# nilsfriess/MultigridMC

Measured on AMD Instinct MI355X. Metric: MGMC V-cycle samples/sec + fine-smoother HBM GB/s, 512³ lattice, 1/2/4/8 GPUs, higher is better.
Workload: dtype f64

## Files before the change

multigridmc_amd/csrc/mgmc_capi.hip:

```cpp
#include "mgmc_internal.hpp"

namespace mgmc_host {
std::mutex g_err_mutex;
std::string g_last_error;
std::atomic<int> g_live_handles{0};
void set_global_error(const std::string& s) {
    std::lock_guard<std::mutex> lock(g_err_mutex);
    g_last_error = s;
}
}

namespace {
constexpr int LDS_POISON_DOUBLES = 80 * 1024 / 8;
__global__ void __launch_bounds__(1024) k_lds_poison() {
    extern __shared__ double lds[];
    const double nan = __builtin_nan("");
    for (int q = threadIdx.x; q < LDS_POISON_DOUBLES; q += blockDim.x) lds[q] = nan;
    __syncthreads();
    if (lds[(threadIdx.x * 7) % LDS_POISON_DOUBLES] == 0.0) asm volatile("" ::: "memory");
}
__global__ void __launch_bounds__(256) k_poison_interior(Layout L, double* __restrict__ x) {
    const int i = blockIdx.x * blockDim.x + threadIdx.x + 1;
    const int j = blockIdx.y + 1;
    const int k = L.dim == 3 ? (int)blockIdx.z + 1 : 0;
// ... 22 lines not shown
    g.seed_hi = (uint32_t)(h->seed >> 32);
    return g;
}

RngKey chain_key_host(const GibbsArg& g, int c) {
    RngKey k = g.key;
    if (c) k.k1 = (g.chain0 + (uint32_t)c) ^ g.seed_hi;
    return k;
}
template <class T>
T* chain_ptr(T* v, const Level& lv, int c) {
    return v ? v + (long long)c * lv.L.nstore : v;
}

template <int DIM, int NPTS, bool NOISE>
void launch_sweep_t(const Level& lv, double* x, const double* f, const GibbsArg& g0, int direction,
                    hipStream_t s) {
    const Layout& L = lv.L;
    const int nc = lv.spec.ncolours;
    dim3 block(64, 4, 1);
    for (int cc = 0; cc < nc; ++cc) {
        GibbsArg g = g0;
        g.colour = (direction == MGMC_FORWARD) ? cc : nc - 1 - cc;
        if (NPTS == 5 || NPTS == 7) {
            dim3 grid = grid3(L.nx / 2, L.ny - 1, DIM == 3 ? L.nz - 1 : 1, block);
            hipLaunchKernelGGL((k_sweep_rb<DIM, NPTS, NOISE>), grid, block, 0, s, L, x, f, lv.S, g);
        } else {
            dim3 grid = grid3(L.nx / 2, L.ny / 2, DIM == 3 ? L.nz / 2 : 1, block);
            hipLaunchKernelGGL((k_sweep_mc<DIM, NPTS, NOISE>), grid, block, 0, s, L, x, f, lv.S, g);
        }
    }
}

void launch_fsweep(const Level& lv, double* x, const double* f, const GibbsArg& g0, int direction, bool noise,
                   hipStream_t s) {
    const Layout& L = lv.L;
    const int nc = lv.F.scheme, dim = lv.spec.dim;
    const int st = nc == 9 || nc == 27 ? 3 : 2;
    dim3 block(64, 4, 1);
    dim3 grid = nc == 2 ? grid3(L.nx / 2, L.ny - 1, dim == 3 ? L.nz - 1 : 1, block)
                        : grid3((L.nx - 1 + st - 1) / st, (L.ny - 1 + st - 1) / st,
                                dim == 3 ? (L.nz - 1 + st - 1) / st : 1, block);
    for (int cc = 0; cc < nc; ++cc) {
        GibbsArg g = g0;
        g.colour = (direction == MGMC_FORWARD) ? cc : nc - 1 - cc;
        if (dim == 3) {
            if (noise) hipLaunchKernelGGL((k_fsweep<3, true>), grid, block, 0, s, L, x, f, lv.F, g);
            else hipLaunchKernelGGL((k_fsweep<3, false>), grid, block, 0, s, L, x, f, lv.F, g);
        } else {
            if (noise) hipLaunchKernelGGL((k_fsweep<2, true>), grid, block, 0, s, L, x, f, lv.F, g);
            else hipLaunchKernelGGL((k_fsweep<2, false>), grid, block, 0, s, L, x, f, lv.F, g);
        }
    }
}

void launch_sweep(const Level& lv, double* x, const double* f, const GibbsArg& g0, int direction, bool noise,
                  hipStream_t s, int nch) {
    if (nch > 1) {
        for (int c = 0; c < nch; ++c) {
            GibbsArg g = g0;
            g.key = chain_key_host(g0, c);
            launch_sweep(lv, chain_ptr(x, lv, c), chain_ptr(f, lv, c), g, direction, noise, s, 1);
        }
        return;
    }
    const GibbsArg& g = g0;
    if (lv.field) {
        launch_fsweep(lv, x, f, g, direction, noise, s);
        return;
    }
    const int dim = lv.spec.dim, np = lv.spec.npoints;
#define DISPATCH(D, P)                                                       \
    if (dim == D && np == P) {                                               \
        if (noise)                                                           \
            launch_sweep_t<D, P, true>(lv, x, f, g, direction, s);           \
        else                                                                 \
            launch_sweep_t<D, P, false>(lv, x, f, g, direction, s);          \
        return;                                                              \
    }
    DISPATCH(3, 7) DISPATCH(3, 27) DISPATCH(2, 5) DISPATCH(2, 9)
#undef DISPATCH
}

template <int XP, int TY, int NT, int MINW = 1>
void launch_zsweep_t(const Level& lv, ZSweepArgs a, bool prolong, hipStream_t s, int nch, bool fz) {
    a.ntx = (lv.L.nx / 2) / XP;
    a.nty = (lv.L.ny - 1 + TY - 1) / TY;
    a.ntz = (lv.L.nz - 1 + a.tz - 1) / a.tz;
    const int ntiles = a.ntx * a.nty * (a.zpairs ? (a.ntz + 1) / 2 * 2 : a.ntz);
    const int nb = (ntiles + 7) / 8 * 8;
    const size_t lds = zsweep_lds_bytes(XP, TY, prolong);
    int ex;
    const bool pow2 = std::isnormal(a.alpha) && std::frexp(std::fabs(a.alpha), &ex) == 0.5 && ex > -900 && ex < 900;
    const dim3 grid(nb, 1, nch);
    const bool lrf = a.lr.e != nullptr;
    if (fz && !lrf) {
        if (prolong && pow2)
            hipLaunchKernelGGL((k_zsweep_rb7<XP, TY, NT, 2, MINW, false, true>), grid, dim3(NT), lds, s, a);
        else if (prolong)
            hipLaunchKernelGGL((k_zsweep_rb7<XP, TY, NT, 1, MINW, false, true>), grid, dim3(NT), lds, s, a);
        else
            hipLaunchKernelGGL((k_zsweep_rb7<XP, TY, NT, 0, MINW, false, true>), grid, dim3(NT), lds, s, a);
        return;
    }
    if (prolong && pow2 && lrf)
        hipLaunchKernelGGL((k_zsweep_rb7<XP, TY, NT, 2, MINW, true>), grid, dim3(NT), lds, s, a);
    else if (prolong && pow2)
        hipLaunchKernelGGL((k_zsweep_rb7<XP, TY, NT, 2, MINW>), grid, dim3(NT), lds, s, a);
    else if (prolong && lrf)
        hipLaunchKernelGGL((k_zsweep_rb7<XP, TY, NT, 1, MINW, true>), grid, dim3(NT), lds, s, a);
    else if (prolong)
        hipLaunchKernelGGL((k_zsweep_rb7<XP, TY, NT, 1, MINW>), grid, dim3(NT), lds, s, a);
    else if (lrf)
        hipLaunchKernelGGL((k_zsweep_rb7<XP, TY, NT, 0, MINW, true>), grid, dim3(NT), lds, s, a);
    else
        hipLaunchKernelGGL((k_zsweep_rb7<XP, TY, NT, 0, MINW>), grid, dim3(NT), lds, s, a);
}

static int zsweep_depth(const Level& lv, int ty, int tzmax) {
    const long long tiles_xy = (long long)((lv.L.nx / 2) / ZS_XP) * ((lv.L.ny - 1 + ty - 1) / ty);
    int tz = tzmax;
    while (tz > 8 && 4 * tiles_xy * ((lv.L.nz - 1 + tz - 1) / tz) < 3LL * 2 * lv.num_cu) tz /= 2;
    return tz;
}

static int zsweep_plain_rows(const Level& lv, int nch) {
    const int tz = zsweep_depth(lv, ZS_TY, ZS_TZ);
    auto ntiles = [&](int ty) {
        const long long nz = (lv.L.nz - 1 + tz - 1) / tz;
        return (long long)((lv.L.nx / 2) / ZS_XP) * ((lv.L.ny - 1 + ty - 1) / ty) * ((nz + 1) / 2 * 2) * nch;
    };
    const long long slots = 2LL * lv.num_cu;
    return (ZS_TYP != ZS_TY && ZS_NTP == ZS_NT && ntiles(ZS_TY) < slots && ntiles(ZS_TYP) <= slots) ? ZS_TYP : ZS_TY;
}

void launch_zsweep(const Level& lv, const double* xin, double* xout, const double* f, const GibbsArg& g0,
                   int direction, const Level* coarse, const double* xc, double alpha, hipStream_t s, int nch = 1,
                   const LRRhsArg* lr = nullptr, bool fzero = false) {
    ZSweepArgs a;
    a.lr = lr ? *lr : LRRhsArg{nullptr};
    a.cs = lv.L.nstore;
    a.csc = coarse ? coarse->L.nstore : 0;
    a.L = lv.L;
    a.xin = xin;
    a.xout = xout;
    a.f = f;
    a.xc = xc;
    a.Lc = coarse ? coarse->L : lv.L;
    a.alpha = alpha;
    a.S = lv.S;
    a.G = g0;
    a.G.colour = (direction == MGMC_FORWARD) ? 0 : 1;
    a.zpairs = 0;
    if (coarse) {
        a.tz = zsweep_depth(lv, ZS_TYP, ZS_TZP);
        launch_zsweep_t<ZS_XP, ZS_TYP, ZS_NTP, ZS_MINWP>(lv, a, true, s, nch, fzero);
        return;
    }
    a.tz = zsweep_depth(lv, ZS_TY, ZS_TZ);
    a.zpairs = 1;
    if (zsweep_plain_rows(lv, nch) != ZS_TY) {
        launch_zsweep_t<ZS_XP, ZS_TYP, ZS_NTP, ZS_MINWP>(lv, a, false, s, nch, fzero);
        return;
    }
    launch_zsweep_t<ZS_XP, ZS_TY, ZS_NT, ZS_MINW>(lv, a, false, s, nch, fzero);
}

bool pairs_eligible(const LevelSpec& sp, const Layout& L) {
    return (sp.npoints == 27 || sp.npoints == 9) && L.nx / 2 >= 1 && L.nx / 2 <= 256 && L.nx % 2 == 0;
}

bool quads_eligible(const LevelSpec& sp, const Layout& L, uint32_t paths) {
    if (!pairs_eligible(sp, L) || (paths & PATH_NO_QUADS)) return false;
    return sp.dim == 2 || L.nx / 2 <= tune::QUADS_MAXPAIR;
}

void launch_rb2d(const Level& lv, const double* xin, double* xout, const double* f, const GibbsArg& g, int direction,
                 bool noise, hipStream_t s, int nch = 1) {
    const int ntx = (lv.L.nx - 1 + RB2_TW - 1) / RB2_TW, nty = (lv.L.ny - 1 + RB2_TH - 1) / RB2_TH;
    const int c1 = direction == MGMC_FORWARD ? 0 : 1;
    const dim3 grid(ntx * nty, 1, nch), block(RB2_NT);
    const long long cs = lv.L.nstore;
    if (noise)
        hipLaunchKernelGGL((k_rb2d<true>), grid, block, 0, s, lv.L, xin, xout, f, lv.S, g, c1, ntx, cs);
    else
        hipLaunchKernelGGL((k_rb2d<false>), grid, block, 0, s, lv.L, xin, xout, f, lv.S, g, c1, ntx, cs);
}

bool jsweep_eligible(const LevelSpec& sp, const Layout& L, uint32_t paths) {
    return sp.dim == 3 && sp.npoints == 27 && (L.nx == 256 || L.nx == 512) &&
           L.ny >= 2 && L.nz >= 2 &&
           !(paths & PATH_NO_JSWEEP);
}


void launch_jsweep(const Level& lv, const double* xin, double* xout, const double* f, const GibbsArg& g, int direction,
                   hipStream_t s, int nch, bool xzero = false) {
    JSweepArgs a;
    a.cs = lv.L.nstore;
    a.L = lv.L;
    a.xo = xin;
    a.xout = xout;
    a.f = f;
    a.S = lv.S;
    a.G = g;
    const int np = lv.L.nx / 2;
    const size_t lds = jsweep_lds_bytes(np);
    const bool fwd = direction == MGMC_FORWARD;
    for (int h = 0; h < 2; ++h) {
        const JSweepPlan p = jsweep_plan(lv.L, fwd, h, lv.num_cu, lds, tune::JS_ROUNDS);
        if (p.nk == 0) continue;
        a.kp = p.kp;
        a.jA = p.jA;
        a.nsteps = p.nsteps;
        a.nk = p.nk;
        a.spc = p.spc;
        a.nchunk = p.nchunk;
        a.xz = h == 0 ? xin : xout;
        const dim3 grid(p.nb, 1, nch), block(2 * np);
#define MGMC_JS_LAUNCH_XZ(NPV, SYMV, XZ)                                                            \
    do {                                                                                            \
        if (fwd) hipLaunchKernelGGL((k_jsweep_half<NPV, false, SYMV, XZ>), grid, block, lds, s, a); \
        else hipLaunchKernelGGL((k_jsweep_half<NPV, true, SYMV, XZ>), grid, block, lds, s, a);      \
    } while (0)
#define MGMC_JS_LAUNCH(NPV, SYMV)                                 \
    do {                                                          \
        if (!xzero) MGMC_JS_LAUNCH_XZ(NPV, SYMV, 0);              \
        else if (h == 0) MGMC_JS_LAUNCH_XZ(NPV, SYMV, 1);         \
        else MGMC_JS_LAUNCH_XZ(NPV, SYMV, 2);                     \
    } while (0)
        if (np == 256) {
            MGMC_JS_LAUNCH(256, false);
        } else if (lv.sym) {
            MGMC_JS_LAUNCH(128, true);
        } else {
            MGMC_JS_LAUNCH(128, false);
        }
#undef MGMC_JS_LAUNCH
#undef MGMC_JS_LAUNCH_XZ
    }
}

void launch_quads(const Level& lv, const double* xin, double* xout, const double* f, const GibbsArg& g, int direction,
                  hipStream_t s, int nch = 1, bool xzero = false, const double2* zb = nullptr) {
    if (lv.jsweep) {
        launch_jsweep(lv, xin, xout, f, g, direction, s, nch, xzero);
        return;
    }
// ... 1968 lines not shown
    const std::string e = validate_operator(*d);
    if (!e.empty()) return fail(nullptr, MGMC_E_INVALID, e);
    const CsrHost A = assemble_operator(*d);
    *nrow = A.nrow;
    *nnz = (int64_t)A.col.size();
    return MGMC_OK;
}

int mgmc_operator_csr(const mgmc_operator_desc* d, int64_t* rowptr, int32_t* col, double* val) {
    if (!d || !rowptr || !col || !val) return fail(nullptr, MGMC_E_INVALID, "null argument");
    const std::string e = validate_operator(*d);
    if (!e.empty()) return fail(nullptr, MGMC_E_INVALID, e);
    const CsrHost A = assemble_operator(*d);
    std::copy(A.rowptr.begin(), A.rowptr.end(), rowptr);
    std::copy(A.col.begin(), A.col.end(), col);
    std::copy(A.val.begin(), A.val.end(), val);
    return MGMC_OK;
}

int mgmc_destroy(mgmc_handle* h) {
    if (!h) return MGMC_OK;
    hipSetDevice(h->device);
    if (h->stream) hipStreamSynchronize(h->stream);
    destroy_graphs(h);
    for (auto e : h->timed_ev0)
        if (e) hipEventDestroy(e);
    free_tails(h);
    for (auto& lv : h->levels) {
        free_lowrank(lv.lr);
        if (lv.x) hipFree(lv.x);
        if (lv.x2) hipFree(lv.x2);
        if (lv.f) hipFree(lv.f);
        if (lv.F.coef && lv.field) hipFree((void*)lv.F.coef);
        if (lv.rbuf) hipFree(lv.rbuf);
        for (auto p : lv.scratch)
            if (p) hipFree(p);
    }
    for (auto p : h->sv)
        if (p) hipFree(p);
    if (h->chol_G) hipFree(h->chol_G);
    if (h->chol_Li) hipFree(h->chol_Li);
    if (h->chol_blk) hipFree(h->chol_blk);
    if (h->sv_scal) hipFree(h->sv_scal);
    if (h->sv_part) hipFree(h->sv_part);
    if (h->comm) ncclCommDestroy(h->comm);
    if (h->tail_prof) hipFree(h->tail_prof);
    if (h->comm_buf) hipFree(h->comm_buf);
    if (h->ctrl) hipFree(h->ctrl);
    if (h->mom) hipFree(h->mom);
    if (h->series) hipFree(h->series);
    if (h->qv_off) hipFree(h->qv_off);
    if (h->qv_val) hipFree(h->qv_val);
    if (h->qv_part) hipFree(h->qv_part);
    if (h->lex_tmp) hipFree(h->lex_tmp);
    if (h->zbuf) hipFree(h->zbuf);
    if (h->stream) hipStreamDestroy(h->stream);
    delete h;
    return MGMC_OK;
}

int mgmc_level_desc_get(const mgmc_handle* h, int level, mgmc_level_desc* out) {
    if (!h || !out) return fail(nullptr, MGMC_E_INVALID, "null argument");
    if (level < 0 || level >= (int)h->levels.size()) return fail(nullptr, MGMC_E_INVALID, "level out of range");
    fill_desc(h->levels[level].spec, out, h->levels[level].field);
    return MGMC_OK;
}

int mgmc_level_kernels(const mgmc_handle* h, int level, char* out, size_t n) {
    if (!h || !out || n == 0) return fail(nullptr, MGMC_E_INVALID, "null argument");
    if (level < 0 || level >= (int)h->levels.size()) return fail(nullptr, MGMC_E_INVALID, "level out of range");
    const Level& lv = h->levels[level];
    const int dim = lv.spec.dim, np = lv.spec.npoints;
    const int tl = tail_level(h);
    const bool last = level + 1 == (int)h->levels.size();
    std::string sweep, post, res;
    if (tl >= 0 && level >= tl) {
        sweep = "k_tail<" + std::to_string(dim) + ">";
    } else if (last) {
        sweep = h->cfg.coarse_solver == MGMC_COARSE_CHOLESKY ? (h->chol_B > 0 ? "k_coarse_chol_blocked" : "k_coarse_chol") : "k_coarse_ssor_lds (or separate colour passes)";
    } else if (lv.field) {
        sweep = "k_fsweep<" + std::to_string(dim) + ">";
    } else if (lv.zsweep) {
        sweep = "k_zsweep_rb7<32," + std::to_string(zsweep_plain_rows(lv, h->nchains)) + ",...,0>";
        if (!(h->paths & PATH_NO_FUSE_PROLONG)) post = "k_zsweep_rb7<32," + std::to_string(tune::ZS_TYP) + ",...,PROLONG>";
    } else if (lv.jsweep) {
        sweep = "k_jsweep_half<" + std::to_string(lv.L.nx / 2) + (lv.sym && lv.L.nx == 256 ? ",sym" : "") + ">";
    } else if (lv.quads) {
        sweep = "k_sweep_quads<" + std::to_string(dim) + ">";
    } else if (lv.rb2d) {
        sweep = "k_rb2d";
    } else if (lv.pairs) {
        sweep = "k_sweep_pairs<" + std::to_string(dim) + ">";
    } else {
        sweep = (np == 2 * dim + 1 ? "k_sweep_rb<" : "k_sweep_mc<") + std::to_string(dim) + ">";
    }
    if (!last && !(tl >= 0 && level >= tl)) {
        const int cx = zrestrict_cx_of(h, level);
        if (lv.field) res = "k_fresidual + k_restrict";
        else if (cx) {
            const Level& lc = h->levels[level + 1];
            const bool wide = np == 7 && cx == 64 &&
                              (long long)((lc.L.nx + 62) / 64) * ((lc.L.ny + 6) / 8) * (lc.L.nz - 1) >= tune::ZR7_WIDE_MIN_TILES;
            res = "k_zresrestrict<" + std::to_string(np) + "," + std::to_string(cx) + "," + (wide ? "8" : "4") + ">";
        } else if (qrestrict_ok(h, level)) {
            sweep = "k_sweep_quads<2> (last pre-sweep: k_quads_restrict2d)";
            res = "k_quads_restrict2d";

        } else res = "k_residual_restrict<" + std::to_string(dim) + "," + std::to_string(np) + ">";
    }
    std::string text = "sweep=" + sweep;
    if (!post.empty()) text += ";post_sweep=" + post;
    bool by_rr = false, by_tail = false;
    for (size_t q = 0; q < h->ops.size(); ++q) {
        const Op& op = h->ops[q];
        if (op.kind != OP_SWEEP || op.level != level || !op.pnz) continue;
        if (q > 0 && h->ops[q - 1].kind == OP_RESIDUAL_RESTRICT && h->ops[q - 1].pn_dst == op.pnz) by_rr = true;
        else by_tail = true;
    }
    if (by_rr || by_tail)
        text += std::string(";noise=") + (by_rr && by_tail ? "restriction+tail" : by_rr ? "restriction" : "tail");
    if (!res.empty()) text += ";residual_restrict=" + res;
    for (const Op& op : h->ops)
        if (op.level == level && op.fzero) {
            text += ";rhs=zero";
            break;
        }
    if (lv.lr.m > 0)
        text += std::string(";lowrank=") + (lv.lr.rhs_inplace ? "dense,rhs_inplace" : lv.lr.dense_path ? "dense"
                                             : lv.lr.small ? "small" : "rows");
    snprintf(out, n, "%s", text.c_str());
    return MGMC_OK;
}

static int put_fine(mgmc_handle* h, double* v, int c, const double* host, size_t n, const char* what) {
    if (!h || !host) return fail(h, MGMC_E_INVALID, "null argument");
    if (n != h->levels[0].spec.ndof) return fail(h, MGMC_E_INVALID, std::string(what) + " size mismatch");
    if (c >= h->nchains) return fail(h, MGMC_E_INVALID, "chain index out of range");
    HIPCHK(h, hipSetDevice(h->device));
    const size_t ns = h->levels[0].L.nstore;
    int rc = upload(h, 0, host, v + (size_t)std::max(c, 0) * ns);
    if (rc) return rc;
    if (c < 0)
        for (int q = 1; q < h->nchains; ++q)
            HIPCHK(h, hipMemcpyAsync(v + q * ns, v, ns * sizeof(double), hipMemcpyDeviceToDevice, h->stream));
    return MGMC_OK;
}

int mgmc_set_rhs(mgmc_handle* h, const double* f, size_t n) {
    int rc = put_fine(h, h ? h->levels[0].f : nullptr, -1, f, n, "rhs");
    if (rc) return rc;
    unsigned long long bits = 0;
    unsigned long long* word = reinterpret_cast<unsigned long long*>(h->ctrl + 7);
    HIPCHK(h, hipMemsetAsync(word, 0, sizeof(*word), h->stream));
    const int nblk = (int)std::min<size_t>((n + 255) / 256, (size_t)16 * h->levels[0].num_cu);
    hipLaunchKernelGGL(k_or_bits, dim3(nblk), dim3(256), 0, h->stream,
                       reinterpret_cast<const unsigned long long*>(h->lex_tmp), (long long)n, word);
    HIPCHK(h, hipGetLastError());
    HIPCHK(h, hipMemcpyAsync(&bits, word, sizeof(bits), hipMemcpyDeviceToHost, h->stream));
    HIPCHK(h, hipStreamSynchronize(h->stream));
    const bool zero = rhs_bits_all_zero(bits);
    if (zero != h->f0_zero) {
        h->f0_zero = zero;
        if (mark_rhs_zero(h)) return build_graphs(h);
    }
    return MGMC_OK;
}

// ... 496 lines not shown
```

multigridmc_amd/csrc/mgmc_internal.hpp:

```cpp
#pragma once
#include <hip/hip_runtime.h>
#include <rccl/rccl.h>
#include <stdio.h>
#include <stdlib.h>
#include <string.h>

#include <algorithm>
#include <atomic>
#include <cmath>
#include <mutex>
#include <string>
#include <vector>

#include "../../include/mgmc.h"
#include "mgmc_hierarchy.hpp"
#include "mgmc_kernels.hpp"
#include "mgmc_zsweep.hpp"
#include "mgmc_tuning.hpp"
#include "mgmc_layout_check.hpp"
static_assert(MGMC_LAYOUT_POINT == mgmc::LF_POINT && MGMC_LAYOUT_PAIRS == mgmc::LF_PAIRS &&
                  MGMC_LAYOUT_ZSWEEP == mgmc::LF_ZSWEEP && MGMC_LAYOUT_ZSWEEP_COARSE == mgmc::LF_ZSWEEP_C &&
                  MGMC_LAYOUT_ZRESTRICT == mgmc::LF_ZRESTRICT && MGMC_LAYOUT_RB2D == mgmc::LF_RB2D &&
                  MGMC_LAYOUT_JSWEEP == mgmc::LF_JSWEEP && MGMC_LAYOUT_QRESTRICT == mgmc::LF_QRESTRICT,
              "layout family bits");
// ... 37 lines not shown
    int src = 0;
    int prolong = 0;
    int lr_next = 0;
    uint32_t lr_next_tag = 0;
    int lr_skip_patch = 0;
    int lr_post_patch = 0;
    uint32_t lr_post_tag = 0;
    int lr_coarse_patch = 0;
    uint32_t lr_coarse_tag = 0;
    int tail = -1;
    int xzero = 0;
    int fzero = 0;
    int zpre = 0;
    const double2* pnz = nullptr;
    double2* pn_dst = nullptr;
    uint32_t pn_tag = 0;
};


enum PathFlag : uint32_t {
    PATH_NO_TAIL = 1u << 0,
    PATH_NO_FUSE_PROLONG = 1u << 1,
    PATH_NO_QUADS = 1u << 2,
    PATH_NO_RB2D = 1u << 3,
    PATH_NO_ZSWEEP = 1u << 4,
    PATH_NO_PAIRS = 1u << 5,
    PATH_NO_ZRESTRICT = 1u << 6,
    PATH_NO_LR_SMALL = 1u << 7,
    PATH_NO_LR_MERGE = 1u << 8,
    PATH_NO_LR_DENSE = 1u << 9,
    PATH_NO_CHOL_DENSE = 1u << 10,
    PATH_NO_JSWEEP = 1u << 11,
    PATH_NO_QRESTRICT = 1u << 12,
    PATH_NO_PROLONG_Z = 1u << 13,
    PATH_NO_XZERO = 1u << 14,
    PATH_NO_FOLD = 1u << 15,
    PATH_NO_POST_NOISE = 1u << 16,
};

struct PathToken {
    const char* name;
    uint32_t flag;
};
constexpr PathToken kPathTokens[] = {
    {"tail", PATH_NO_TAIL},           {"fuse_prolong", PATH_NO_FUSE_PROLONG},
    {"quads", PATH_NO_QUADS},         {"rb2d", PATH_NO_RB2D},
    {"zsweep", PATH_NO_ZSWEEP},       {"pairs", PATH_NO_PAIRS},
    {"zrestrict", PATH_NO_ZRESTRICT}, {"lr_small", PATH_NO_LR_SMALL},
    {"lr_merge", PATH_NO_LR_MERGE},   {"lr_dense", PATH_NO_LR_DENSE},
    {"chol_dense", PATH_NO_CHOL_DENSE}, {"jsweep", PATH_NO_JSWEEP},
    {"qrestrict", PATH_NO_QRESTRICT}, {"prolong_z", PATH_NO_PROLONG_Z},
    {"xzero", PATH_NO_XZERO},         {"fold", PATH_NO_FOLD},
    {"post_noise", PATH_NO_POST_NOISE},
};

inline bool read_path_flags(uint32_t* flags, std::string* bad) {
    *flags = 0;
    const char* e = getenv("MGMC_DISABLE");
    if (!e) return true;
    std::string list(e);
    size_t pos = 0;
    while (pos <= list.size()) {
        size_t end = list.find(',', pos);
        if (end == std::string::npos) end = list.size();
        const std::string tok = list.substr(pos, end - pos);
        if (!tok.empty()) {
            bool found = false;
            for (const PathToken& t : kPathTokens)
                if (tok == t.name) {
                    *flags |= t.flag;
                    found = true;
                }
            if (!found) {
                *bad = tok;
                return false;
            }
        }
        pos = end + 1;
    }
    return true;
}

constexpr int ZS_XP = 32, ZS_TY = tune::ZS_TY, ZS_NT = zs_threads(ZS_TY), ZS_MINW = tune::ZS_MINW,
              ZS_TZ = tune::ZS_TZ, ZS_TYP = tune::ZS_TYP, ZS_NTP = zs_threads(ZS_TYP),
              ZS_MINWP = tune::ZS_MINWP, ZS_TZP = tune::ZS_TZP;

struct LowRankDev {
    int m = 0;
    int nblk = 0;
    LRColMeta* meta = nullptr;
    int* blk_col = nullptr;
    LRBlock* blk = nullptr;
    long long* ent_off = nullptr;
    double* ent_val = nullptr;
    double* dense_val = nullptr;
    int nrows = 0;
    long long* rows_off = nullptr;
    double* rows_coef = nullptr;
    uint64_t* rows_mask = nullptr;
    double* save = nullptr;
    int nbar[2] = {0, 0};
    long long* bar_off[2] = {nullptr, nullptr};
    double* bar_val[2] = {nullptr, nullptr};
    double* sc_one = nullptr;
    double* sc_inv = nullptr;
    double* sq = nullptr;
    double* part = nullptr;
    double* w = nullptr;
    bool small = false;
    long long max_col_n = 0;
    int* t_ent_off = nullptr;
    int* t_rows_off = nullptr;
    int* t_bar_off[2] = {nullptr, nullptr};
    bool dense_path = false;
    bool dense_const = false;
    double dense_cval = 0.0;
    int dense_slot = 0;
    int dense_g = -1;
    uint32_t* skip_b = nullptr;
    uint32_t* skip_y[2] = {nullptr, nullptr};
    double* yg[2] = {nullptr, nullptr};
    uint8_t* ykey = nullptr;
    double* ytab[2] = {nullptr, nullptr};
    double* minv_g[2] = {nullptr, nullptr};
    double* fe = nullptr;
    double* fe2 = nullptr;
    bool rhs_inplace = false;
    double* rhs_e = nullptr;
    int split_g = -1;
    long long nbar_all[2] = {0, 0};
    std::vector<void*> allocs;
};

struct Level {
    LevelSpec spec;
    Layout L;
    StencilArg S;
    double* x = nullptr;
    double* x2 = nullptr;
    double* f = nullptr;
    double* scratch[3] = {nullptr, nullptr, nullptr};
    size_t lds_bytes = 0;
    int num_cu = 256;
    uint32_t paths = 0;
    bool zsweep = false;
    bool pairs = false;
    bool quads = false;
    bool jsweep = false;
    bool rb2d = false;
    bool field = false;
    bool sym = false;
    bool fold = false;
    FieldArg F;
    double* rbuf = nullptr;
    bool pingpong() const { return zsweep || quads || rb2d; }
    double* buf(int i) const { return i == 0 ? x : x2; }
    LowRankDev lr;
};

inline void free_lowrank(LowRankDev& lr) {
    for (void* p : lr.allocs) hipFree(p);
    lr = LowRankDev();
}

extern std::atomic<int> g_live_handles;
struct LiveHandleCount {
    LiveHandleCount() { g_live_handles.fetch_add(1); }
    ~LiveHandleCount() { g_live_handles.fetch_sub(1); }
// ... 148 lines not shown
```

multigridmc_amd/csrc/mgmc_tuning.hpp:

```cpp
#pragma once

namespace mgmc {
namespace tune {

constexpr int ZS_TY = 20;
constexpr int ZS_MINW = 6;
constexpr int ZS_TZ = 32;
constexpr int ZS_TYP = 16;
constexpr int ZS_MINWP = 6;
constexpr int ZS_TZP = 128;

constexpr int QUADS_MAXPAIR = 64;
constexpr int QUADS_NT = 128;
constexpr int QUADS_NT_WIDE = 256;
constexpr int QUADS_NT3 = 128;
constexpr int QUADS_LANES = 1;

constexpr int JS_D = 3;
constexpr int JS_ROUNDS = 1;

constexpr int ZR27_CX = 64;
constexpr int ZR27_CY = 4;
constexpr int ZR27_MINW = 1;
constexpr int ZR_SMALL_NX = 32;
constexpr int ZR7_WIDE_MIN_TILES = 16 * 1024;

constexpr int PROLONG_Z = 8;
constexpr int PROLONG_Z_SMALL = 4;

constexpr int TAIL_PN_WG = 32;

constexpr int LR_STAGED_MAX_WAVES = 512;
constexpr int LR_PART_U = 8;
constexpr int LR_PART_CH = 1;
constexpr int LR_DENSE_PER = 8;

}
}
```

multigridmc_amd/csrc/mgmc_zsweep.hpp:

```cpp
#pragma once
#include <type_traits>

#include "mgmc_kernels.hpp"
#include "mgmc_tuning.hpp"

namespace mgmc {

struct ZSweepArgs {
    Layout L;
    const double* xin;
    double* xout;
    const double* f;
    const double* xc;
    Layout Lc;
    double alpha;
    StencilArg S;
    GibbsArg G;
    int tz;
    int ntx, nty, ntz;
    int zpairs;
    long long cs, csc;
    LRRhsArg lr;
};

struct ZItem {
    int goff;
    uint32_t pbase;
    int lds;
    int flags;
};

struct RunE0 {
    int value;
};

constexpr int zs_threads(int TY) { return 256 * ((TY / 2 + 2 + 3) / 4); }

template <int XP, int TY, int NT, int PROLONG, int MINW, bool LRF = false, bool FZ = false>
__global__ void __launch_bounds__(NT) __attribute__((amdgpu_waves_per_eu(MINW))) k_zsweep_rb7(ZSweepArgs a) {
    static_assert(XP == 32 && TY % 4 == 0 && TY <= 32 && NT == zs_threads(TY), "tile shape");
    static_assert(!(LRF && FZ), "a patched right-hand side is not zero");
    constexpr int WP = XP + 2;
    constexpr int RS = 2 * WP + 2;
    constexpr int R = TY + 4;
    constexpr int PS = R * RS;
    constexpr int NSLOT = 4;
    constexpr int NCW = TY / 2;
    constexpr int NLX = (R * WP + NT - 1) / NT;
    extern __shared__ __attribute__((aligned(16))) double smem[];
    double* xs = smem;
    double* tab = xs + NSLOT * PS;
    for (int q = threadIdx.x; q < 64; q += NT) {
        tab[q] = LOGTAB_RC[q];
        tab[64 + q] = LOGTAB_HI[q];
        tab[128 + q] = LOGTAB_LO[q];
    }
    for (int q = threadIdx.x; q < 130; q += NT) tab[192 + q] = SINCOS_TAB[q];
    if (!PROLONG) __syncthreads();
    constexpr int CW = XP + 8, CWP = CW / 2, CR = TY / 2 + 3, CPS = CR * CW;
    constexpr int NLC = PROLONG ? (CR * CWP + NT - 1) / NT : 1;
    double* cring = tab + 322;

    {
        const int ch = batch_chain();
        a.xin += ch * a.cs;
        a.xout += ch * a.cs;
        if (!FZ) a.f += ch * a.cs;
        if (PROLONG) a.xc += ch * a.csc;
        a.G.key = chain_key(a.G, ch);
        if (LRF) a.lr.e += ch;
    }
    const double lre = LRF ? *a.lr.e : 0.0;
    const Layout& L = a.L;
    const int nb = gridDim.x;
    const int b = blockIdx.x;
    const int per = nb >> 3;
    const int tile = (nb & 7) ? b : (b & 7) * per + (b >> 3);
    int txi = tile % a.ntx;
    int tyi = (tile / a.ntx) % a.nty;
    int tzi = tile / (a.ntx * a.nty);
    bool down = false;
    if (!PROLONG && a.zpairs) {
        const int nxy = a.ntx * a.nty;
        const int zp = tile / (2 * nxy), rem = tile - zp * 2 * nxy;
        txi = (rem >> 1) % a.ntx;
        tyi = (rem >> 1) / a.ntx;
        tzi = 2 * zp + (rem & 1);
        down = (rem & 1) != 0;
    }
    if (tzi >= a.ntz) return;
    const int q0 = txi * XP;
    const int j0 = 1 + tyi * TY;
    const int k0 = 1 + tzi * a.tz;
    const int k1 = min(k0 + a.tz, L.nz);
    const int ibase = 2 * q0 - 1;
    const int fc = a.G.colour;
    const double sd = a.G.sd, wd = a.G.wd;
    const uint64_t sample = *a.G.sample;
    const uint32_t s_lo = (uint32_t)sample, s_hi = (uint32_t)(sample >> 32);
    const uint32_t plane_pairs = (uint32_t)((uint64_t)(L.ny - 1) * (uint64_t)(L.nx / 2));
    const int tid = threadIdx.x;
    const int wave = __builtin_amdgcn_readfirstlane(tid >> 6), lane = tid & 63;

    auto slot = [](int p) { return (p + 4) & 3; };
    auto interior_plane = [&](int k) { return k >= 1 && k <= L.nz - 1; };
    auto make_item = [&](int r, int c2) {
        ZItem t;
        const int j = j0 - 2 + r, i = ibase + 2 * c2;
        const bool rin = j >= 1 && j <= L.ny - 1;
        const int jc = j < 0 ? 0 : (j > L.ny ? L.ny : j);
        t.goff = (int)((long long)jc * L.sx + i + L.off);
        t.pbase = (uint32_t)((uint64_t)(j - 1) * (uint64_t)(L.nx / 2) + (uint64_t)((i - 1) >> 1));
        t.lds = r * RS + c2;
        t.flags = (rin ? 1 : 0) | ((i >= 1 && i <= L.nx - 1) ? 2 : 0) | ((i + 1 >= 1 && i + 1 <= L.nx - 1) ? 4 : 0) |
                  (((i + j) & 1) << 3);
        return t;
    };

    const bool core_wave = wave < NCW, active_wave = wave < NCW + 2;
    int ir = 2, ic = 1;
    if (core_wave) {
        ir = 2 + 4 * (wave >> 1) + (wave & 1) + (lane >= 32 ? 2 : 0);
        ic = 1 + (lane & 31);
    } else if (active_wave) {
        const int h = wave - NCW;
        const int l = (lane < 32 + TY) ? lane : 0;
        if (l < 32) {
            ir = h == 0 ? 1 : R - 2;
            ic = 1 + l;
        } else {
            const int m = l - 32;
            ir = (h == 0 ? 3 : 2) + 2 * (m >> 1);
            ic = (m & 1) ? WP - 1 : 0;
        }
    }
    const ZItem t = make_item(ir, ic);
    const int wpar = __builtin_amdgcn_readfirstlane((t.flags >> 3) & 1);
    const int E0 = __builtin_amdgcn_readfirstlane(((wpar ^ (k0 - 1)) & 1) == fc ? 0 : 1);
    const int E0d = __builtin_amdgcn_readfirstlane(((wpar ^ k1) & 1) == fc ? 0 : 1);
    const bool rowin = (t.flags & 1) != 0;
    const bool in0 = rowin && (t.flags & 2), in1 = rowin && (t.flags & 4);

    int xoff[NLX];
    int xlds[NLX];
#pragma unroll
    for (int u = 0; u < NLX; ++u) {
        const int it = tid + u * NT;
        xoff[u] = L.off + 1;
        xlds[u] = -1;
        if (it < R * WP) {
            constexpr int NE = (R + 1) / 2;
            const int r = it < NE * WP ? 2 * (it / WP) : 2 * ((it - NE * WP) / WP) + 1;
            const ZItem q = make_item(r, it % WP);
            xlds[u] = q.lds;
            xoff[u] = q.goff;
        }
    }
    int pcro[NLX];
    auto plane_base = [&](const double* v, int k) { return v + (long long)(k < 0 ? 0 : (k > L.nz ? L.nz : k)) * L.sp; };

    const Layout& Lc = a.Lc;
    const int Jst = (j0 - 2) >> 1;
    int coff[NLC], clds[NLC];
    double2 pcv[NLC];
#pragma unroll
    for (int u = 0; u < NLC; ++u) {
        const int it = tid + u * NT;
        clds[u] = (PROLONG && it < CR * CWP) ? 2 * it : -1;
        const int r = it / CWP, c = 2 * (it % CWP);
        const int jr = Jst + r;
        const int jc = jr < 0 ? 0 : (jr > Lc.ny ? Lc.ny : jr);
        coff[u] = clds[u] >= 0 ? (int)((long long)jc * Lc.sx + (q0 - 3 + c) + Lc.off) : Lc.off + 1;
    }
    auto issue_c = [&](int K) {
        const double* base = a.xc + (long long)(K < 0 ? 0 : (K > Lc.nz ? Lc.nz : K)) * Lc.sp;
#pragma unroll
        for (int u = 0; u < NLC; ++u) pcv[u] = *reinterpret_cast<const double2*>(base + coff[u]);
    };
    auto deposit_c = [&](int K) {
        double* dst = cring + (K & 1) * CPS;
#pragma unroll
        for (int u = 0; u < NLC; ++u)
            if (clds[u] >= 0) {
                dst[clds[u]] = pcv[u].x;
                dst[clds[u] + 1] = pcv[u].y;
            }
    };
    const double al0 = a.alpha, al1 = a.alpha * 0.5;
    auto prolong_pair = [&](double2 v, int jodd, int k, int cro, auto KO) {
        const int K0 = k >> 1;
        const int kodd = decltype(KO)::value >= 0 ? decltype(KO)::value : (k & 1);
        const double awx = ldexp(al1, -(jodd + kodd)), awy = ldexp(al0, -(jodd + kodd));
        const double* cp0 = cring + cro;
#pragma unroll
        for (int aa = 0; aa < 2; ++aa) {
            if (aa == 1 && !kodd) break;
            const double* cp = cp0 + ((K0 + aa) & 1) * CPS;
#pragma unroll
            for (int bb = 0; bb < 2; ++bb) {
                if (bb == 1 && !jodd) break;
                const double c0 = cp[bb * CW], c1 = cp[bb * CW + 1];
                if (PROLONG == 2) {
                    v.x = fma(awx, c0, v.x);
                    v.x = fma(awx, c1, v.x);
                    v.y = fma(awy, c1, v.y);
                } else {
                    v.x = v.x + awx * c0;
                    v.x = v.x + awx * c1;
                    v.y = v.y + awy * c1;
                }
            }
        }
        return v;
    };

#pragma unroll
    for (int u = 0; u < NLX; ++u) {
        const int c2 = xlds[u] < 0 ? 0 : xlds[u] % RS, j = xlds[u] < 0 ? j0 : j0 - 2 + xlds[u] / RS;
        pcro[u] = 2 * (c2 + 2 + ((j >> 1) - Jst) * CW) + (j & 1);
    }

    constexpr bool PF2 = PROLONG != 0;
    double2 pxb[PF2 ? 2 : 1][NLX];
#define ZS_PX(B) pxb[PF2 ? (B) : 0]
    auto issue_x = [&](int k, auto Bc) {
        const double* base =
            plane_base(a.xin, k > k1 + 1 ? k1 + 1 : (k < k0 - 2 ? k0 - 2 : k));
#pragma unroll
        for (int u = 0; u < NLX; ++u) ZS_PX(decltype(Bc)::value)[u] = *reinterpret_cast<const double2*>(base + xoff[u]);
    };
    auto deposit_x = [&](int k, auto KO, auto Bc) {
        double* dst = xs + slot(k) * PS;
#pragma unroll
        for (int u = 0; u < NLX; ++u) {
            if (xlds[u] < 0) continue;
            double2 v = ZS_PX(decltype(Bc)::value)[u];
            if (PROLONG && interior_plane(k)) v = prolong_pair(v, pcro[u] & 1, k, pcro[u] >> 1, KO);
            dst[xlds[u]] = v.x;
            dst[xlds[u] + WP] = v.y;
        }
    };
    const int foff = PF2 ? (active_wave ? t.goff : L.off + 1) : t.goff;
    auto load_f = [&](int k) {
        return *reinterpret_cast<const double2*>(
            plane_base(a.f, k > k1 ? k1 : (k < k0 - 1 ? k0 - 1 : k)) + foff);
    };

    const double cz = a.S.a[4], cy = a.S.a[10], cx = a.S.a[12], cc = a.S.a[13];
    auto row_sum = [&](int k, int o, int e, double below) {
        const double* s0 = xs + slot(k) * PS;
        const double* sp = xs + slot(k + 1) * PS;
        const int xm = e ? o - WP : o + WP - 1;
        double res = cz * below;
        res = fma(cy, s0[o - RS], res);
        res = fma(cx, s0[xm], res);
        res = fma(cc, s0[o], res);
        res = fma(cx, s0[xm + 1], res);
        res = fma(cy, s0[o + RS], res);
        res = fma(cz, sp[o], res);
        return res;
    };
    auto row_sum_ba = [&](int k, int o, int e, double below, double above) {
        const double* s0 = xs + slot(k) * PS;
        const int xm = e ? o - WP : o + WP - 1;
        double res = cz * below;
        res = fma(cy, s0[o - RS], res);
        res = fma(cx, s0[xm], res);
        res = fma(cc, s0[o], res);
        res = fma(cx, s0[xm + 1], res);
        res = fma(cy, s0[o + RS], res);
        res = fma(cz, above, res);
        return res;
    };
    auto noise = [&](int k) -> double2 {
        const uint32_t pair = (uint32_t)(k - 1) * plane_pairs + t.pbase;
        uint32_t key0 = a.G.key.k0, key1 = a.G.key.k1;
        asm volatile("" : "+s"(key0), "+s"(key1));
        const Philox4 rnd = philox4x32_10(pair, a.G.tag, s_lo, s_hi, key0, key1);
        double z0, z1;
        normal_pair_t(rnd, &z0, &z1, tab, tab + 64, tab + 128, tab + 192);
        return make_double2(z0, z1);
    };
    double2 z = make_double2(0.0, 0.0);
    double fb = 0.0;
    auto run = [&](auto E0c, auto DNc) __attribute__((always_inline)) {
        const int E0c_v = E0c.value;
        constexpr bool DN = decltype(DNc)::value;
        constexpr int dz = DN ? -1 : 1;
        auto step = [&](int p, auto ODDc, double2& fcur, double2& fnxt, double pk_in, double& pk_out)
                        __attribute__((always_inline)) {
            constexpr bool odd_step = decltype(ODDc)::value;
            const int e = odd_step ? 1 - E0c_v : E0c_v;
            const int o1 = t.lds + e * WP, o2 = t.lds + (1 - e) * WP;
            const bool inf = e ? in1 : in0;
            using Bp = std::integral_constant<int, odd_step ? 0 : 1>;
            deposit_x(p + dz, std::integral_constant<int, DN ? -1 : (odd_step ? 0 : 1)>{}, Bp{});
            if (PROLONG) {
                if (odd_step) deposit_c((p + 3) / 2);
                else issue_c((p + 4) / 2);
            }
            if constexpr (PF2) {
                issue_x(p + 3, Bp{});
                (void)fnxt;
            } else {
                issue_x(p + 2 * dz, Bp{});
                if constexpr (!FZ) {
                    if (active_wave) fnxt = load_f(p + dz);
                }
            }
            __syncthreads();
            if (interior_plane(p) && active_wave) {
                double2 fv = make_double2(0.0, 0.0);
                if constexpr (!FZ) fv = fcur;
                if constexpr (LRF) fv = lr_rhs_pair(fv, lre);
                if (inf) {
                    const double res = row_sum(p, o1, e, xs[slot(p - 1) * PS + o1]);
                    const double crhs = fma(sd, e ? z.y : z.x, e ? fv.y : fv.x);
                    double* s0 = xs + slot(p) * PS;
                    s0[o1] = fma(wd, crhs - res, s0[o1]);
                }
                pk_out = fma(sd, e ? z.x : z.y, e ? fv.x : fv.y);
            }
            if constexpr (PF2 && !FZ) fcur = load_f(p + 2);
            __syncthreads();
            const int k = p - dz;
            if (core_wave) {
                const bool own = k >= k0 && k < k1;
                const double* s0 = xs + slot(k) * PS;
                const double fv = s0[o2];
                if (own && rowin) {
                    double sv = s0[o1];
                    if (inf) {
                        const double res = DN ? row_sum_ba(k, o1, e, xs[slot(p) * PS + o1], fb) : row_sum(k, o1, e, fb);
                        sv = fma(wd, pk_in - res, sv);
                    }
                    double* dst = a.xout + (long long)k * L.sp + t.goff;
                    const double2 out = e ? make_double2(fv, sv) : make_double2(sv, fv);
                    __builtin_nontemporal_store(out.x, dst);
                    __builtin_nontemporal_store(out.y, dst + 1);
                }
                fb = fv;
            }
            if (active_wave && interior_plane(p + dz)) z = noise(p + dz);
        };
        double2 fA = make_double2(0.0, 0.0), fB = make_double2(0.0, 0.0);
        double pkA = 0.0, pkB = 0.0;
        const int pst = DN ? k1 : k0 - 1;
        if constexpr (FZ) {
        } else if constexpr (PF2) {
            fA = load_f(k0 - 1);
            fB = load_f(k0);
        } else if (active_wave) {
            fA = load_f(pst);
        }
        if (active_wave && interior_plane(pst)) z = noise(pst);
        if constexpr (DN) {
            for (int p = k1; p >= k0 - 1; p -= 2) {
                step(p, std::integral_constant<bool, false>{}, fA, fB, pkB, pkA);
                if (p - 1 >= k0 - 1) step(p - 1, std::integral_constant<bool, true>{}, fB, fA, pkA, pkB);
            }
        } else {
            for (int p = k0 - 1; p <= k1; p += 2) {
                step(p, std::integral_constant<bool, false>{}, fA, fB, pkB, pkA);
                if (p + 1 <= k1) step(p + 1, std::integral_constant<bool, true>{}, fB, fA, pkA, pkB);
            }
        }
    };

    if (PROLONG) {
        issue_c((k0 - 3) / 2);
        deposit_c((k0 - 3) / 2);
        issue_c((k0 - 1) / 2);
        deposit_c((k0 - 1) / 2);
        __syncthreads();
    }
    using B0 = std::integral_constant<int, 0>;
    using B1 = std::integral_constant<int, 1>;
    using UP = std::integral_constant<bool, false>;
    using DOWN = std::integral_constant<bool, true>;
    if (!PROLONG && down) {
        issue_x(k1 + 1, B1{});
        deposit_x(k1 + 1, std::integral_constant<int, -1>{}, B1{});
        issue_x(k1, B0{});
        deposit_x(k1, std::integral_constant<int, -1>{}, B0{});
        issue_x(k1 - 1, B1{});
        if (E0d) run(std::integral_constant<int, 1>{}, DOWN{});
        else run(std::integral_constant<int, 0>{}, DOWN{});
        return;
    }
    issue_x(k0 - 2, B1{});
    deposit_x(k0 - 2, std::integral_constant<int, -1>{}, B1{});
    issue_x(k0 - 1, B0{});
    deposit_x(k0 - 1, std::integral_constant<int, -1>{}, B0{});
    if (PROLONG) {
        __syncthreads();
        issue_c((k0 + 1) / 2);
        deposit_c((k0 + 1) / 2);
        __syncthreads();
    }
    issue_x(k0, B1{});
    if constexpr (PF2) issue_x(k0 + 1, B0{});
    if (PROLONG) run(RunE0{E0}, UP{});
    else if (E0) run(std::integral_constant<int, 1>{}, UP{});
    else run(std::integral_constant<int, 0>{}, UP{});
}

#undef ZS_PX

inline size_t zsweep_lds_bytes(int XP, int TY, bool prolong) {
    const int RS = 2 * (XP + 2) + 2, R = TY + 4;
    const int coarse = prolong ? 2 * (TY / 2 + 3) * (XP + 8) : 0;
    return (size_t)(4 * R * RS + 3 * 64 + 130 + coarse) * sizeof(double);
}

}
```

Measured before the change: 498.4.

## Add overflow-wave staging and taller fzero prolong tiles to z-sweep

Adds a staging plan for the prolongation z-sweep: when the tile's load items leave a small remainder of at most one wave, wave 0 loads that remainder through a separate overflow register pipeline instead of every thread carrying an extra load slot. It also adds a separate tile shape (20 rows, depth 86) for the fused-prolong zero-RHS sweep, chosen by occupancy heuristics, and keeps depth halving even. The aim is to cut register pressure and wasted staging work and to better fill CUs. The cost is more template variants and an imbalanced wave 0, and the odd tile sizes may lower efficiency.

```diff
diff --git a/multigridmc_amd/csrc/mgmc_capi.hip b/multigridmc_amd/csrc/mgmc_capi.hip
--- a/multigridmc_amd/csrc/mgmc_capi.hip
+++ b/multigridmc_amd/csrc/mgmc_capi.hip
@@ -128,45 +128,38 @@
 #undef DISPATCH
 }
 
-template <int XP, int TY, int NT, int MINW = 1>
-void launch_zsweep_t(const Level& lv, ZSweepArgs a, bool prolong, hipStream_t s, int nch, bool fz) {
-    a.ntx = (lv.L.nx / 2) / XP;
-    a.nty = (lv.L.ny - 1 + TY - 1) / TY;
+template <class K>
+static void launch_zsweep_k(K kernel, const Level& lv, ZSweepArgs a, int ty, int nt, bool prolong, hipStream_t s, int nch) {
+    a.ntx = (lv.L.nx / 2) / ZS_XP;
+    a.nty = (lv.L.ny - 1 + ty - 1) / ty;
     a.ntz = (lv.L.nz - 1 + a.tz - 1) / a.tz;
     const int ntiles = a.ntx * a.nty * (a.zpairs ? (a.ntz + 1) / 2 * 2 : a.ntz);
     const int nb = (ntiles + 7) / 8 * 8;
-    const size_t lds = zsweep_lds_bytes(XP, TY, prolong);
+    const dim3 grid(nb, 1, nch);
+    hipLaunchKernelGGL(kernel, grid, dim3(nt), zsweep_lds_bytes(ZS_XP, ty, prolong), s, a);
+}
+
+template <int TY, int MINW>
+static void launch_zsweep_plain(const Level& lv, const ZSweepArgs& a, hipStream_t s, int nch, bool fz) {
+    constexpr int NT = zs_threads(TY);
+    if (a.lr.e) launch_zsweep_k(k_zsweep_rb7<ZS_XP, TY, NT, 0, MINW, true>, lv, a, TY, NT, false, s, nch);
+    else if (fz) launch_zsweep_k(k_zsweep_rb7<ZS_XP, TY, NT, 0, MINW, false, true>, lv, a, TY, NT, false, s, nch);
+    else launch_zsweep_k(k_zsweep_rb7<ZS_XP, TY, NT, 0, MINW>, lv, a, TY, NT, false, s, nch);
+}
+
+template <int TY, int MINW, bool LRF, bool FZ>
+static void launch_zsweep_post(const Level& lv, const ZSweepArgs& a, hipStream_t s, int nch) {
+    constexpr int NT = zs_threads(TY);
     int ex;
     const bool pow2 = std::isnormal(a.alpha) && std::frexp(std::fabs(a.alpha), &ex) == 0.5 && ex > -900 && ex < 900;
-    const dim3 grid(nb, 1, nch);
-    const bool lrf = a.lr.e != nullptr;
-    if (fz && !lrf) {
-        if (prolong && pow2)
-            hipLaunchKernelGGL((k_zsweep_rb7<XP, TY, NT, 2, MINW, false, true>), grid, dim3(NT), lds, s, a);
-        else if (prolong)
-            hipLaunchKernelGGL((k_zsweep_rb7<XP, TY, NT, 1, MINW, false, true>), grid, dim3(NT), lds, s, a);
-        else
-            hipLaunchKernelGGL((k_zsweep_rb7<XP, TY, NT, 0, MINW, false, true>), grid, dim3(NT), lds, s, a);
-        return;
-    }
-    if (prolong && pow2 && lrf)
-        hipLaunchKernelGGL((k_zsweep_rb7<XP, TY, NT, 2, MINW, true>), grid, dim3(NT), lds, s, a);
-    else if (prolong && pow2)
-        hipLaunchKernelGGL((k_zsweep_rb7<XP, TY, NT, 2, MINW>), grid, dim3(NT), lds, s, a);
-    else if (prolong && lrf)
-        hipLaunchKernelGGL((k_zsweep_rb7<XP, TY, NT, 1, MINW, true>), grid, dim3(NT), lds, s, a);
-    else if (prolong)
-        hipLaunchKernelGGL((k_zsweep_rb7<XP, TY, NT, 1, MINW>), grid, dim3(NT), lds, s, a);
-    else if (lrf)
-        hipLaunchKernelGGL((k_zsweep_rb7<XP, TY, NT, 0, MINW, true>), grid, dim3(NT), lds, s, a);
-    else
-        hipLaunchKernelGGL((k_zsweep_rb7<XP, TY, NT, 0, MINW>), grid, dim3(NT), lds, s, a);
+    if (pow2) launch_zsweep_k(k_zsweep_rb7<ZS_XP, TY, NT, 2, MINW, LRF, FZ>, lv, a, TY, NT, true, s, nch);
+    else launch_zsweep_k(k_zsweep_rb7<ZS_XP, TY, NT, 1, MINW, LRF, FZ>, lv, a, TY, NT, true, s, nch);
 }
 
 static int zsweep_depth(const Level& lv, int ty, int tzmax) {
     const long long tiles_xy = (long long)((lv.L.nx / 2) / ZS_XP) * ((lv.L.ny - 1 + ty - 1) / ty);
     int tz = tzmax;
-    while (tz > 8 && 4 * tiles_xy * ((lv.L.nz - 1 + tz - 1) / tz) < 3LL * 2 * lv.num_cu) tz /= 2;
+    while (tz > 8 && 4 * tiles_xy * ((lv.L.nz - 1 + tz - 1) / tz) < 3LL * 2 * lv.num_cu) tz = std::max(8, (tz / 2) & ~1);
     return tz;
 }
 
@@ -176,8 +169,17 @@
         const long long nz = (lv.L.nz - 1 + tz - 1) / tz;
         return (long long)((lv.L.nx / 2) / ZS_XP) * ((lv.L.ny - 1 + ty - 1) / ty) * ((nz + 1) / 2 * 2) * nch;
     };
-    const long long slots = 2LL * lv.num_cu;
-    return (ZS_TYP != ZS_TY && ZS_NTP == ZS_NT && ntiles(ZS_TY) < slots && ntiles(ZS_TYP) <= slots) ? ZS_TYP : ZS_TY;
+    if (ZS_TYS == ZS_TY || zs_threads(ZS_TYS) != ZS_NT) return ZS_TY;
+    return zs_pick_rows(ntiles(ZS_TY), ntiles(ZS_TYS), 2LL * lv.num_cu, ZS_TY, ZS_TYS);
+}
+
+static int zsweep_post_rows(const Level& lv, int nch, bool fz) {
+    if (!fz || ZS_TYPZ == ZS_TYP) return ZS_TYP;
+    const int tz = zsweep_depth(lv, ZS_TYP, ZS_TZP);
+    auto ntiles = [&](int ty) {
+        return (long long)((lv.L.nx / 2) / ZS_XP) * ((lv.L.ny - 1 + ty - 1) / ty) * ((lv.L.nz - 1 + tz - 1) / tz) * nch;
+    };
+    return zs_pick_rows(ntiles(ZS_TYPZ), ntiles(ZS_TYP), 2LL * lv.num_cu, ZS_TYPZ, ZS_TYP);
 }
 
 void launch_zsweep(const Level& lv, const double* xin, double* xout, const double* f, const GibbsArg& g0,
@@ -198,18 +200,23 @@
     a.G = g0;
     a.G.colour = (direction == MGMC_FORWARD) ? 0 : 1;
     a.zpairs = 0;
+    const bool fz = fzero && !a.lr.e;
     if (coarse) {
+        if (zsweep_post_rows(lv, nch, fz) != ZS_TYP) {
+            a.tz = zsweep_depth(lv, ZS_TYPZ, ZS_TZPZ);
+            launch_zsweep_post<ZS_TYPZ, ZS_MINWP, false, true>(lv, a, s, nch);
+            return;
+        }
         a.tz = zsweep_depth(lv, ZS_TYP, ZS_TZP);
-        launch_zsweep_t<ZS_XP, ZS_TYP, ZS_NTP, ZS_MINWP>(lv, a, true, s, nch, fzero);
+        if (a.lr.e) launch_zsweep_post<ZS_TYP, ZS_MINWP, true, false>(lv, a, s, nch);
+        else if (fz) launch_zsweep_post<ZS_TYP, ZS_MINWP, false, true>(lv, a, s, nch);
+        else launch_zsweep_post<ZS_TYP, ZS_MINWP, false, false>(lv, a, s, nch);
         return;
     }
     a.tz = zsweep_depth(lv, ZS_TY, ZS_TZ);
     a.zpairs = 1;
-    if (zsweep_plain_rows(lv, nch) != ZS_TY) {
-        launch_zsweep_t<ZS_XP, ZS_TYP, ZS_NTP, ZS_MINWP>(lv, a, false, s, nch, fzero);
-        return;
-    }
-    launch_zsweep_t<ZS_XP, ZS_TY, ZS_NT, ZS_MINW>(lv, a, false, s, nch, fzero);
+    if (zsweep_plain_rows(lv, nch) != ZS_TY) launch_zsweep_plain<ZS_TYS, ZS_MINWP>(lv, a, s, nch, fz);
+    else launch_zsweep_plain<ZS_TY, ZS_MINW>(lv, a, s, nch, fz);
 }
 
 bool pairs_eligible(const LevelSpec& sp, const Layout& L) {
@@ -2344,7 +2351,11 @@
         sweep = "k_fsweep<" + std::to_string(dim) + ">";
     } else if (lv.zsweep) {
         sweep = "k_zsweep_rb7<32," + std::to_string(zsweep_plain_rows(lv, h->nchains)) + ",...,0>";
-        if (!(h->paths & PATH_NO_FUSE_PROLONG)) post = "k_zsweep_rb7<32," + std::to_string(tune::ZS_TYP) + ",...,PROLONG>";
+        if (!(h->paths & PATH_NO_FUSE_PROLONG)) {
+            bool fz = false;
+            for (const Op& op : h->ops) fz = fz || (op.kind == OP_SWEEP && op.level == level && op.prolong && op.fzero && lv.lr.m == 0);
+            post = "k_zsweep_rb7<32," + std::to_string(zsweep_post_rows(lv, h->nchains, fz)) + ",...,PROLONG>";
+        }
     } else if (lv.jsweep) {
         sweep = "k_jsweep_half<" + std::to_string(lv.L.nx / 2) + (lv.sym && lv.L.nx == 256 ? ",sym" : "") + ">";
     } else if (lv.quads) {
diff --git a/multigridmc_amd/csrc/mgmc_internal.hpp b/multigridmc_amd/csrc/mgmc_internal.hpp
--- a/multigridmc_amd/csrc/mgmc_internal.hpp
+++ b/multigridmc_amd/csrc/mgmc_internal.hpp
@@ -143,8 +143,8 @@
 }
 
 constexpr int ZS_XP = 32, ZS_TY = tune::ZS_TY, ZS_NT = zs_threads(ZS_TY), ZS_MINW = tune::ZS_MINW,
-              ZS_TZ = tune::ZS_TZ, ZS_TYP = tune::ZS_TYP, ZS_NTP = zs_threads(ZS_TYP),
-              ZS_MINWP = tune::ZS_MINWP, ZS_TZP = tune::ZS_TZP;
+              ZS_TZ = tune::ZS_TZ, ZS_TYS = tune::ZS_TYS, ZS_TYP = tune::ZS_TYP, ZS_MINWP = tune::ZS_MINWP,
+              ZS_TZP = tune::ZS_TZP, ZS_TYPZ = tune::ZS_TYPZ, ZS_TZPZ = tune::ZS_TZPZ;
 
 struct LowRankDev {
     int m = 0;
diff --git a/multigridmc_amd/csrc/mgmc_tuning.hpp b/multigridmc_amd/csrc/mgmc_tuning.hpp
--- a/multigridmc_amd/csrc/mgmc_tuning.hpp
+++ b/multigridmc_amd/csrc/mgmc_tuning.hpp
@@ -9,6 +9,9 @@
 constexpr int ZS_TYP = 16;
 constexpr int ZS_MINWP = 6;
 constexpr int ZS_TZP = 128;
+constexpr int ZS_TYPZ = 20;
+constexpr int ZS_TZPZ = 86;
+constexpr int ZS_TYS = 16;
 
 constexpr int QUADS_MAXPAIR = 64;
 constexpr int QUADS_NT = 128;
diff --git a/multigridmc_amd/csrc/mgmc_zstage.hpp b/multigridmc_amd/csrc/mgmc_zstage.hpp
--- /dev/null
+++ b/multigridmc_amd/csrc/mgmc_zstage.hpp
@@ -0,0 +1,30 @@
+#pragma once
+
+namespace mgmc {
+
+struct ZStagePlan {
+    int slots;
+    int nov;
+};
+
+constexpr ZStagePlan zs_stage_plan(int R, int WP, int NT) {
+    const int items = R * WP, full = items / NT, rest = items % NT;
+    if (full >= 1 && rest > 0 && rest <= 64) return ZStagePlan{full, rest};
+    return ZStagePlan{(items + NT - 1) / NT, 0};
+}
+
+struct ZStageRC {
+    int r, c2;
+};
+
+constexpr ZStageRC zs_stage_item(int R, int WP, int it) {
+    const int NE = (R + 1) / 2;
+    const int r = it < NE * WP ? 2 * (it / WP) : 2 * ((it - NE * WP) / WP) + 1;
+    return ZStageRC{r, it % WP};
+}
+
+constexpr int zs_pick_rows(long long tiles_tall, long long tiles_short, long long slots, int tall, int shrt) {
+    return (tiles_tall < slots && tiles_short <= slots) ? shrt : tall;
+}
+
+}
diff --git a/multigridmc_amd/csrc/mgmc_zsweep.hpp b/multigridmc_amd/csrc/mgmc_zsweep.hpp
--- a/multigridmc_amd/csrc/mgmc_zsweep.hpp
+++ b/multigridmc_amd/csrc/mgmc_zsweep.hpp
@@ -3,6 +3,7 @@
 
 #include "mgmc_kernels.hpp"
 #include "mgmc_tuning.hpp"
+#include "mgmc_zstage.hpp"
 
 namespace mgmc {
 
@@ -46,7 +47,9 @@
     constexpr int PS = R * RS;
     constexpr int NSLOT = 4;
     constexpr int NCW = TY / 2;
-    constexpr int NLX = (R * WP + NT - 1) / NT;
+    constexpr ZStagePlan PLAN = PROLONG != 0 ? zs_stage_plan(R, WP, NT) : ZStagePlan{(R * WP + NT - 1) / NT, 0};
+    constexpr int NLX = PLAN.slots, NOV = PLAN.nov;
+    constexpr bool OVF = NOV > 0;
     extern __shared__ __attribute__((aligned(16))) double smem[];
     double* xs = smem;
     double* tab = xs + NSLOT * PS;
@@ -149,12 +152,18 @@
         xoff[u] = L.off + 1;
         xlds[u] = -1;
         if (it < R * WP) {
-            constexpr int NE = (R + 1) / 2;
-            const int r = it < NE * WP ? 2 * (it / WP) : 2 * ((it - NE * WP) / WP) + 1;
-            const ZItem q = make_item(r, it % WP);
+            const ZStageRC rc = zs_stage_item(R, WP, it);
+            const ZItem q = make_item(rc.r, rc.c2);
             xlds[u] = q.lds;
             xoff[u] = q.goff;
         }
+    }
+    int ovoff = L.off + 1, ovlds = 0;
+    if (OVF) {
+        const ZStageRC rc = zs_stage_item(R, WP, NLX * NT + (lane < NOV ? lane : 0));
+        const ZItem q = make_item(rc.r, rc.c2);
+        ovlds = q.lds;
+        ovoff = q.goff;
     }
     int pcro[NLX];
     auto plane_base = [&](const double* v, int k) { return v + (long long)(k < 0 ? 0 : (k > L.nz ? L.nz : k)) * L.sp; };
@@ -219,6 +228,11 @@
         const int c2 = xlds[u] < 0 ? 0 : xlds[u] % RS, j = xlds[u] < 0 ? j0 : j0 - 2 + xlds[u] / RS;
         pcro[u] = 2 * (c2 + 2 + ((j >> 1) - Jst) * CW) + (j & 1);
     }
+    int ovpcro = 0;
+    if (OVF && PROLONG) {
+        const int c2 = ovlds % RS, j = j0 - 2 + ovlds / RS;
+        ovpcro = 2 * (c2 + 2 + ((j >> 1) - Jst) * CW) + (j & 1);
+    }
 
     constexpr bool PF2 = PROLONG != 0;
     double2 pxb[PF2 ? 2 : 1][NLX];
@@ -239,6 +253,18 @@
             dst[xlds[u]] = v.x;
             dst[xlds[u] + WP] = v.y;
         }
+    };
+    double2 pov = make_double2(0.0, 0.0);
+    auto issue_ov = [&](int k) {
+        const double* base = plane_base(a.xin, k > k1 + 1 ? k1 + 1 : (k < k0 - 2 ? k0 - 2 : k));
+        pov = *reinterpret_cast<const double2*>(base + ovoff);
+    };
+    auto deposit_ov = [&](int k, auto KO) {
+        double* dst = xs + slot(k) * PS;
+        double2 v = pov;
+        if (PROLONG && interior_plane(k)) v = prolong_pair(v, ovpcro & 1, k, ovpcro >> 1, KO);
+        dst[ovlds] = v.x;
+        dst[ovlds + WP] = v.y;
     };
     const int foff = PF2 ? (active_wave ? t.goff : L.off + 1) : t.goff;
     auto load_f = [&](int k) {
@@ -294,7 +320,14 @@
             const int o1 = t.lds + e * WP, o2 = t.lds + (1 - e) * WP;
             const bool inf = e ? in1 : in0;
             using Bp = std::integral_constant<int, odd_step ? 0 : 1>;
-            deposit_x(p + dz, std::integral_constant<int, DN ? -1 : (odd_step ? 0 : 1)>{}, Bp{});
+            using KOp = std::integral_constant<int, DN ? -1 : (odd_step ? 0 : 1)>;
+            deposit_x(p + dz, KOp{}, Bp{});
+            if constexpr (OVF) {
+                if (wave == 0) {
+                    deposit_ov(p + dz, KOp{});
+                    issue_ov(p + 2 * dz);
+                }
+            }
             if (PROLONG) {
                 if (odd_step) deposit_c((p + 3) / 2);
                 else issue_c((p + 4) / 2);
@@ -378,20 +411,30 @@
     using B1 = std::integral_constant<int, 1>;
     using UP = std::integral_constant<bool, false>;
     using DOWN = std::integral_constant<bool, true>;
+    using KX = std::integral_constant<int, -1>;
+    auto stage_now = [&](int k, auto Bc) {
+        issue_x(k, Bc);
+        deposit_x(k, KX{}, Bc);
+        if constexpr (OVF) {
+            if (wave == 0) {
+                issue_ov(k);
+                deposit_ov(k, KX{});
+            }
+        }
+    };
     if (!PROLONG && down) {
-        issue_x(k1 + 1, B1{});
-        deposit_x(k1 + 1, std::integral_constant<int, -1>{}, B1{});
-        issue_x(k1, B0{});
-        deposit_x(k1, std::integral_constant<int, -1>{}, B0{});
+        stage_now(k1 + 1, B1{});
+        stage_now(k1, B0{});
         issue_x(k1 - 1, B1{});
+        if constexpr (OVF) {
+            if (wave == 0) issue_ov(k1 - 1);
+        }
         if (E0d) run(std::integral_constant<int, 1>{}, DOWN{});
         else run(std::integral_constant<int, 0>{}, DOWN{});
         return;
     }
-    issue_x(k0 - 2, B1{});
-    deposit_x(k0 - 2, std::integral_constant<int, -1>{}, B1{});
-    issue_x(k0 - 1, B0{});
-    deposit_x(k0 - 1, std::integral_constant<int, -1>{}, B0{});
+    stage_now(k0 - 2, B1{});
+    stage_now(k0 - 1, B0{});
     if (PROLONG) {
         __syncthreads();
         issue_c((k0 + 1) / 2);
@@ -400,6 +443,9 @@
     }
     issue_x(k0, B1{});
     if constexpr (PF2) issue_x(k0 + 1, B0{});
+    if constexpr (OVF) {
+        if (wave == 0) issue_ov(k0);
+    }
     if (PROLONG) run(RunE0{E0}, UP{});
     else if (E0) run(std::integral_constant<int, 1>{}, UP{});
     else run(std::integral_constant<int, 0>{}, UP{});
```

New measurement: 500.6 (median of 6 runs). About the same (+0.4%).
